# springmeyer/cov-tiles

Measured on AMD Instinct MI355X. Metric: GB/s raw COVT bytes decoded + Mvertices/s, z2–z14 tile batch, 1/2/4/8 GPU, higher is better.
Workload: dtype int32

## Files before the change

### cov-tiles_amd/csrc/covt_decode.hip

```cpp
#include <hip/hip_runtime.h>
#include <stdint.h>

#include "covt.h"
#include "covt_internal.h"
#include "covt_wave.h"
#include "covt_walk.h"

namespace covt {

constexpr int kWin = 1024;

#ifndef COVT_LONG_STREAM
#define COVT_LONG_STREAM 16384
#endif
#ifndef COVT_LONG_PRIO
#define COVT_LONG_PRIO 2
#endif
#ifndef COVT_RLE_SHORT_SPAN
#define COVT_RLE_SHORT_SPAN 448
#endif
#ifndef COVT_CHUNK_PRIO
#define COVT_CHUNK_PRIO 2
#endif
constexpr int kLongStream = COVT_LONG_STREAM;
// ... 142 lines not shown
#else
    __builtin_nontemporal_store(w, (i32x4*)p);
#endif
}
template <class T>
__device__ __forceinline__ void st_out(T* p, T v) {
#if defined(COVT_ABL_NOSTORE)
    *(T*)((uintptr_t)p & ~(uintptr_t)1023) = v;
#else
    *p = v;
#endif
}
__device__ __forceinline__ int64_t pack_xy(int32_t x, int32_t y) {
    return (int64_t)(((uint64_t)(uint32_t)y << 32) | (uint32_t)x);
}

template <int E>
__device__ __forceinline__ void store_run(uint8_t* arr, int32_t o, int32_t n, int64_t base, int32_t delta) {
    constexpr int K = 16 / E;
    const int l = lane_id();
    auto val = [&](int32_t i) -> int64_t { return (int64_t)((uint64_t)base + (uint64_t)(int64_t)(int32_t)(i * delta)); };
    const int32_t a0 = (o + K - 1) & ~(K - 1);
    const int32_t head = min(a0 - o, n);
    const int32_t nch = (n - head) / K;
    const int32_t body_end = head + nch * K;
    const int32_t ti = l < head ? l : body_end + (l - head);
    if (l < head || (l - head < n - body_end && l >= head)) {
        const int64_t v = val(ti);
        if (E == 8) st_out((int64_t*)arr + o + ti, v);
        else if (E == 4) st_out((int32_t*)arr + o + ti, (int32_t)v);
        else st_out(arr + o + ti, (uint8_t)v);
    }
    for (int32_t c0 = 0; c0 < nch; c0 += 64) {
        const int32_t ch = c0 + l < nch ? c0 + l : nch - 1;
        const int32_t i = head + K * ch;
        int4 w;
        if (E == 8) {
            const int64_t v0 = val(i), v1 = val(i + 1);
            w = make_int4((int)v0, (int)(v0 >> 32), (int)v1, (int)(v1 >> 32));
        } else if (E == 4) {
            w = make_int4((int)val(i), (int)val(i + 1), (int)val(i + 2), (int)val(i + 3));
        } else {
            const uint32_t b = (uint32_t)base & 0xffu, q = b * 0x01010101u;
            w = make_int4((int)q, (int)q, (int)q, (int)q);
        }
        st_out16((int32_t*)(arr + (int64_t)(o + i) * E), w);
    }
}

template <int E>
__device__ __forceinline__ void store_run_q(uint8_t* arr, int32_t o, int32_t n, int64_t base, int32_t delta) {
    constexpr int K = 16 / E;
    static_assert(2 * (K - 1) <= 16, "head and tail elements fit a quarter");
    const int q = lane_id() & 15;
    auto val = [&](int32_t i) -> int64_t { return (int64_t)((uint64_t)base + (uint64_t)(int64_t)(int32_t)(i * delta)); };
    const int32_t a0 = (o + K - 1) & ~(K - 1);
    const int32_t head = n > 0 ? min(a0 - o, n) : 0;
    const int32_t nch = n > 0 ? (n - head) / K : 0;
    const int32_t body_end = head + nch * K;
    const int32_t tailn = n > 0 ? n - body_end : 0;
    if (q < head + tailn) {
        const int32_t ti = q < head ? q : body_end + (q - head);
        const int64_t v = val(ti);
        if (E == 8) st_out((int64_t*)arr + o + ti, v);
        else st_out((int32_t*)arr + o + ti, (int32_t)v);
    }
    const int32_t steps = (int32_t)wave_max((uint32_t)((nch + 15) >> 4));
    for (int32_t c0 = 0; c0 < 16 * steps; c0 += 16) {
        const int32_t ch = c0 + q;
        if (ch < nch) {
            const int32_t i = head + K * ch;
            int4 w;
            if (E == 8) {
                const int64_t v0 = val(i), v1 = val(i + 1);
                w = make_int4((int)v0, (int)(v0 >> 32), (int)v1, (int)(v1 >> 32));
            } else {
                w = make_int4((int)val(i), (int)val(i + 1), (int)val(i + 2), (int)val(i + 3));
            }
            st_out16((int32_t*)(arr + (int64_t)(o + i) * E), w);
        }
    }
}

template <int OP, int K>
__device__ __forceinline__ void sink_values(const uint32_t (&vin)[K], int64_t base, int32_t first, int32_t count,
                                            int nb, uint8_t* __restrict__ out, Carry& c) {
    const int l = lane_id();
    const bool full = first == 0 && count >= 64 * K;
    const int32_t s0 = l * K - first;
    const bool lfull = full || (s0 >= 0 && s0 + K <= count);
    const int64_t i0 = base + (int64_t)l * K;
    bool ok[K];
    uint32_t v[K];
#pragma unroll
    for (int k = 0; k < K; ++k) {
        ok[k] = full || (s0 + k >= 0 && s0 + k < count);
        v[k] = ok[k] ? vin[k] : 0u;
    }
    auto st32 = [&](const int32_t (&r)[K]) {
        int32_t* o = (int32_t*)out + i0;
        if (K == 4 && lfull) {
            st_out16(o, make_int4(r[0], r[K > 1 ? 1 : 0], r[K > 2 ? 2 : 0], r[K > 3 ? 3 : 0]));
        } else {
#pragma unroll
            for (int k = 0; k < K; ++k)
                if (ok[k]) st_out(o + k, r[k]);
        }
    };
    auto st64 = [&](const int64_t (&r)[K]) {
        int64_t* o = (int64_t*)out + i0;
#pragma unroll
        for (int k = 0; k < K; ++k)
            if (ok[k]) st_out(o + k, r[k]);
    };
    if constexpr (OP == COVT_OP_VARINT_I32 || OP == COVT_OP_VARINT_ZZ_I32) {
        int32_t r[K];
#pragma unroll
        for (int k = 0; k < K; ++k) r[k] = OP == COVT_OP_VARINT_I32 ? (int32_t)v[k] : zz32(v[k]);
        st32(r);
    } else if constexpr (OP == COVT_OP_VARINT_I32_AS_I64 || OP == COVT_OP_VARINT_ZZ_I32_AS_I64) {
        int64_t r[K];
#pragma unroll
        for (int k = 0; k < K; ++k) r[k] = OP == COVT_OP_VARINT_I32_AS_I64 ? (int64_t)(int32_t)v[k] : (int64_t)zz32(v[k]);
        st64(r);
    } else if constexpr (OP == COVT_OP_VARINT_ZZ_DELTA_I32 || OP == COVT_OP_FPF_ZZ_DELTA_I32 ||
                         OP == COVT_OP_VARINT_ZZ_DELTA_I64) {
        uint32_t sacc[K];
        uint32_t acc = 0;
#pragma unroll
        for (int k = 0; k < K; ++k) {
            acc += (uint32_t)zz32(v[k]);
            sacc[k] = acc;
        }
        const uint32_t inc = incl_scan(acc);
        const uint32_t pre = c.x + inc - acc;
        if constexpr (OP == COVT_OP_VARINT_ZZ_DELTA_I64) {
            int64_t r[K];
#pragma unroll
            for (int k = 0; k < K; ++k) r[k] = (int64_t)(int32_t)(pre + sacc[k]);
            st64(r);
        } else {
            int32_t r[K];
#pragma unroll
            for (int k = 0; k < K; ++k) r[k] = (int32_t)(pre + sacc[k]);
            st32(r);
        }
        c.x += lane_bcast(inc, 63);
    } else if constexpr (OP == COVT_OP_VARINT_ZZ_DELTA_XY || OP == COVT_OP_FPF_ZZ_DELTA_XY) {
        uint32_t sx[K], sy[K];
        uint32_t ax = 0, ay = 0;
        const uint32_t par0 = (uint32_t)(i0 & 1);
#pragma unroll
        for (int k = 0; k < K; ++k) {
            const uint32_t z = (uint32_t)zz32(v[k]);
            const bool isx = ((par0 + k) & 1u) == 0;
            ax += isx ? z : 0u;
            ay += isx ? 0u : z;
            sx[k] = ax;
            sy[k] = ay;
        }
        const uint32_t incx = incl_scan(ax), incy = incl_scan(ay);
        const uint32_t prex = c.x + incx - ax, prey = c.y + incy - ay;
        int32_t r[K];
#pragma unroll
        for (int k = 0; k < K; ++k) r[k] = (int32_t)((((par0 + k) & 1u) == 0) ? (prex + sx[k]) : (prey + sy[k]));
        st32(r);
        c.x += lane_bcast(incx, 63);
        c.y += lane_bcast(incy, 63);
    } else if constexpr (OP == COVT_OP_VARINT_DELTA_MORTON || OP == COVT_OP_FPF_DELTA_MORTON) {
        uint32_t sacc[K];
        uint32_t acc = 0;
#pragma unroll
        for (int k = 0; k < K; ++k) {
            acc += v[k];
            sacc[k] = acc;
        }
        const uint32_t inc = incl_scan(acc);
        const uint32_t pre = c.x + inc - acc;
        const int32_t half = morton_half(nb);
        int32_t* o = (int32_t*)out + 2 * i0;
        int32_t xy[2 * K];
#pragma unroll
        for (int k = 0; k < K; ++k) {
            uint32_t mx, my;
            morton_xy((int32_t)(pre + sacc[k]), nb, mx, my);
            xy[2 * k] = (int32_t)(mx - (uint32_t)half);
            xy[2 * k + 1] = (int32_t)(my - (uint32_t)half);
        }
        if (K == 4 && lfull) {
            st_out16(o, make_int4(xy[0], xy[1], xy[K > 1 ? 2 : 0], xy[K > 1 ? 3 : 0]));
            st_out16(o + 4, make_int4(xy[K > 2 ? 4 : 0], xy[K > 2 ? 5 : 0], xy[K > 3 ? 6 : 0], xy[K > 3 ? 7 : 0]));
        } else {
#pragma unroll
            for (int k = 0; k < K; ++k)
                if (ok[k]) st_out((int64_t*)(o + 2 * k), pack_xy(xy[2 * k], xy[2 * k + 1]));
        }
        c.x += lane_bcast(inc, 63);
    }
}

enum { MODE_RAW = 0, MODE_WORDREV = 1 };
enum { VAL_J4 = 0, VAL_VB = 1, VAL_U64 = 2, VAL_U64_STRICT = 3, VAL_NONE = 4 };

__device__ __forceinline__ uint32_t win_byte(const WaveSmem& sm, int32_t j) {
    return ((const uint8_t*)sm.u.v.win)[j];
}
__device__ __forceinline__ void win_bytes12(const WaveSmem& sm, int32_t j, uint32_t& x0, uint32_t& x1,
                                            uint32_t& x2) {
    const int32_t d = j >> 2;
    const uint32_t sh = (uint32_t)(j & 3);
    const uint32_t w0 = sm.u.v.win[d], w1 = sm.u.v.win[d + 1], w2 = sm.u.v.win[d + 2], w3 = sm.u.v.win[d + 3];
    x0 = __builtin_amdgcn_alignbyte(w1, w0, sh);
    x1 = __builtin_amdgcn_alignbyte(w2, w1, sh);
    x2 = __builtin_amdgcn_alignbyte(w3, w2, sh);
}

struct Win {
    int32_t woff;
    int32_t K;
    int32_t p0;
    bool valid, serial;
    uint4 d;
    uint32_t cpre, cmsk;
};

template <int MODE, int VAL>
__device__ void win_load(WaveSmem& sm, const uint8_t* sb, Win& w, int32_t p, int32_t end, const uint32_t* lsrc = nullptr,
                         int32_t lw0 = 0) {
    const int l = lane_id();
    uint4 d;
    int32_t woff;
    if (MODE == MODE_RAW) {
        const uintptr_t a = ((uintptr_t)(sb + p)) & ~(uintptr_t)15;
        woff = uni((int32_t)((intptr_t)a - (intptr_t)sb));
        d = woff + 16 * l < end ? ld128(a + 16 * (uintptr_t)l) : make_uint4(0, 0, 0, 0);
    } else {
        woff = p & ~15;
        const uint8_t* q = sb + woff + 16 * l;
        d = make_uint4(0, 0, 0, 0);
        if (woff + 16 * l < end) {
            if (lsrc) {
                const uint32_t* ws = lsrc + ((woff + 16 * l) >> 2) - lw0;
                d = make_uint4(ws[0], ws[1], ws[2], ws[3]);
            } else {
                d.x = ld_be32(q);
                d.y = ld_be32(q + 4);
                d.z = ld_be32(q + 8);
                d.w = ld_be32(q + 12);
            }
        }
        wave_sync();
    }
    ((uint4*)sm.u.v.win)[l] = d;
    if (VAL == VAL_NONE) {
        wave_sync();
        w.d = d;
        w.woff = woff;
        w.K = 0;
        w.p0 = p;
        w.valid = true;
        w.serial = false;
        return;
    }
    const int32_t q0 = woff + 16 * l;
    const uint32_t V = range16((VAL == VAL_J4 ? p : 0) - q0, end - q0);
    const uint32_t H = hibits16(d);
    uint32_t T = (VAL == VAL_VB) ? (V & H) : (V & ~H);
    bool serial = false;
    if (VAL == VAL_J4) {
        const uint32_t N = V & ~T;
        uint32_t prevN = (uint32_t)__shfl_up((int)N, 1, 64);
        if (l == 0) prevN = 0;
        const uint32_t ext = (N << 3) | ((prevN >> 13) & 7u);
        serial = __any((ext & (ext >> 1) & (ext >> 2) & (ext >> 3)) != 0);
    }
    int32_t K;
    if (!serial) {
        const uint32_t cnt = __popc(T);
        const uint32_t inc = incl_scan(cnt);
        uint32_t idx = inc - cnt;
        sm.cpre[l] = (uint16_t)idx;
// ... 3 lines not shown
        while (T) {
            const int k = __ffs(T) - 1;
            T &= T - 1;
            sm.u.v.list[idx++] = (uint16_t)(16 * l + k);
        }
        K = (int32_t)lane_bcast(inc, 63);
    } else {
        wave_sync();
        if (l == 0) {
            const int32_t lim = (end < woff + kWin ? end : woff + kWin) - woff;
            int32_t j = p - woff, k = 0;
            while (j < lim) {
                int32_t len = 0;
                bool done = false;
                for (int b = 0; b < 4; ++b) {
                    if (j + b >= lim) break;
                    ++len;
                    if (b == 3 || (win_byte(sm, j + b) & 0x80u) == 0) { done = true; break; }
                }
                if (!done) break;
                sm.u.v.list[k++] = (uint16_t)(j + len - 1);
                j += len;
            }
            sm.misc[0] = k;
        }
        wave_sync();
        K = uni(sm.misc[0]);
    }
    wave_sync();
    w.d = d;
    w.woff = woff;
    w.K = K;
    w.p0 = p;
    w.valid = true;
    w.serial = serial || VAL == VAL_J4;
}

__device__ __forceinline__ int32_t win_rank(const WaveSmem& sm, const Win& w, int32_t q) {
    const int32_t j = q - w.woff;
    if (j <= 0) return 0;
    if (j >= kWin) return w.K;
    const int32_t c = j >> 4;
    return (int32_t)uniu((uint32_t)sm.cpre[c] + __popc((uint32_t)sm.cmask[c] & ((1u << (j & 15)) - 1u)));
}

template <int VAL>
__device__ __forceinline__ void win_value(const WaveSmem& sm, int32_t sj, int32_t ej, uint32_t& lo, uint32_t& hi,
                                          bool& lerr) {
    const int32_t len = ej - sj + 1;
    uint32_t x0, x1, x2;
    win_bytes12(sm, sj, x0, x1, x2);
    lo = 0;
    hi = 0;
    if (VAL == VAL_J4) {
        lo = pext7(x0 & bytemask(len));
    } else if (VAL == VAL_VB) {
        if (len <= 5) {
            lo = pext7(x0 & bytemask(len));
            if (len == 5) lo += (x1 & 0x7fu) << 28;
        } else {
            uint32_t vv = 0;
            for (int b = 0; b < len; ++b) vv += (win_byte(sm, sj + b) & 0x7fu) << ((7 * b) & 31);
            lo = vv;
        }
    } else {
        uint64_t rv;
        if (len <= 10) {
            const uint32_t m0 = x0 & bytemask(len), m1 = x1 & bytemask(len - 4), m2 = x2 & bytemask(len - 8);
            rv = (uint64_t)pext7(m0) | ((uint64_t)pext7(m1) << 28) | ((uint64_t)(m2 & 0x7fu) << 56) |
                 ((uint64_t)((m2 >> 8) & 0x7fu) << 63);
        } else {
            rv = 0;
            for (int b = 0; b < len; ++b) rv |= (uint64_t)(win_byte(sm, sj + b) & 0x7fu) << ((7 * b) & 63);
            lerr = true;
        }
        lo = (uint32_t)rv;
        hi = (uint32_t)(rv >> 32);
    }
}

#ifndef COVT_VARINT_LINES
#define COVT_VARINT_LINES 1
#endif
template <int MODE, int VAL, int K = 1, class Emit>
__device__ int32_t varint_take(WaveSmem& sm, const uint8_t* sb, Win& w, int32_t& pos, int32_t end, int32_t want,
                               bool until_end, int32_t& err, Emit&& emit, int32_t out0 = 0,
                               int32_t* first_bad = nullptr, int32_t line = 0, const uint32_t* lsrc = nullptr,
                               int32_t lw0 = 0) {
    const int l = lane_id();
    int32_t got = 0;
    while (until_end ? (pos < end) : (got < want)) {
        if (!w.valid || pos < w.woff || pos >= w.woff + kWin || (w.serial && pos != w.p0)) {
            win_load<MODE, VAL>(sm, sb, w, pos, end, lsrc, lw0);
            lsrc = nullptr;
        }
        const int32_t r = w.serial ? 0 : win_rank(sm, w, pos);
        const int32_t have = w.K - r;
        if (have <= 0) {
            const int32_t aligned = (MODE == MODE_RAW) ? (int32_t)(((uintptr_t)(sb + pos) & ~(uintptr_t)15) -
                                                                   (uintptr_t)sb)
                                                       : (pos & ~15);
            if (w.woff != aligned) {
                win_load<MODE, VAL>(sm, sb, w, pos, end);
                continue;
            }
            if (until_end) break;
            err = (w.woff + kWin >= end) ? COVT_ERR_TRUNCATED : COVT_ERR_BAD_HEADER;
            break;
        }
        int32_t take = have;
        if (until_end) {
            if (got + have > want) { err = COVT_ERR_COUNT_MISMATCH; take = want - got; }
        } else if (take > want - got) {
            take = want - got;
        }
        if (take <= 0) break;
        if (COVT_VARINT_LINES && MODE == MODE_RAW && line && !until_end && got + take < want) {
            const int32_t cut = (out0 + got + take) & (line - 1);
            if (cut < take) {
                take -= cut;
            } else {
                const int32_t aligned = (int32_t)(((uintptr_t)(sb + pos) & ~(uintptr_t)15) - (uintptr_t)sb);
                if (w.woff != aligned) {
                    win_load<MODE, VAL>(sm, sb, w, pos, end);
                    continue;
                }
            }
        }
        bool lerr = false;
        int32_t fb = INT32_MAX;
        const int32_t s0 = pos - w.woff;
        const int32_t lead = (K > 1) ? ((out0 + got) & (K - 1)) : 0;
        for (int32_t g = -lead; g < take; g += 64 * K) {
            uint32_t lo[K], hi[K];
#pragma unroll
            for (int k = 0; k < K; ++k) {
                int32_t vi = g + K * l + k;
                vi = vi < 0 ? 0 : (vi < take ? vi : take - 1);
                const int32_t li = r + vi - 1;
                const int32_t pv = (int32_t)sm.u.v.list[li < 0 ? 0 : li] + 1;
                const int32_t sj = vi == 0 ? s0 : pv;
                if constexpr (VAL == VAL_J4) {
                    const int32_t dq = sj >> 2;
                    const uint32_t x = __builtin_amdgcn_alignbyte(sm.u.v.win[dq + 1], sm.u.v.win[dq], (uint32_t)sj & 3u);
                    const uint32_t u = ~x & 0x80808080u;
                    lo[k] = pext7(x & (u ^ (u - 1u)));
                    hi[k] = 0;
                } else {
                    bool lk = false;
                    win_value<VAL>(sm, sj, sm.u.v.list[r + vi], lo[k], hi[k], lk);
                    if (VAL == VAL_U64_STRICT && first_bad && lk) fb = min(fb, got + vi);
                    lerr = lerr || lk;
                }
            }
            const int32_t first = g < 0 ? -g : 0;
            const int32_t cnt = (take - g < 64 * K ? take - g : 64 * K) - first;
            emit(lo, hi, got + g, first, cnt);
        }
        if (VAL == VAL_U64_STRICT && __any(lerr) && !err) {
            err = COVT_ERR_BAD_HEADER;
            if (first_bad) *first_bad = (int32_t)~wave_max(~(uint32_t)fb);
        }
        pos = w.woff + (int32_t)uniu(sm.u.v.list[r + take - 1]) + 1;
        if (w.serial) { w.p0 = pos; w.valid = false; }
        got += take;
        if (err) break;
    }
    return got;
}

struct Ctx {
    WaveSmem* sm;
    const uint8_t* sb;
    uint8_t* out;
    int32_t avail, n, nb, op, byte_length;
    int32_t err, consumed;
#ifdef COVT_TIMING
    uint64_t ph_last;
    uint32_t ph[kPhases];
#endif
};
#ifdef COVT_TIMING
#define COVT_PHASE(c, k)                                          \
    do {                                                          \
        const uint64_t t_ = __builtin_amdgcn_s_memtime();         \
        (c).ph[k] += (uint32_t)(t_ - (c).ph_last);                \
        (c).ph_last = t_;                                         \
    } while (0)
#else
#define COVT_PHASE(c, k) \
    do {                 \
    } while (0)
#endif

template <int VAL>
__device__ __forceinline__ uint32_t rd_byte(Ctx& c, Win& w, int32_t q, int32_t need = 1) {
    if (!w.valid || q < w.woff || (q + need > w.woff + kWin && w.woff + kWin < c.avail))
        win_load<MODE_RAW, VAL>(*c.sm, c.sb, w, q, c.avail);
    return uniu(win_byte(*c.sm, q - w.woff));
}

template <int OP>
__device__ __forceinline__ void sink_u64(const uint32_t (&lo)[4], const uint32_t (&hi)[4], int64_t base, int32_t first,
                                         int32_t count, int64_t* o, uint64_t& acc) {
    const int32_t s0 = 4 * lane_id() - first;
    int64_t* p = o + base + 4 * lane_id();
    uint64_t v[4];
#pragma unroll
    for (int k = 0; k < 4; ++k) {
        const bool ok = s0 + k >= 0 && s0 + k < count;
        v[k] = ok ? (((uint64_t)hi[k] << 32) | lo[k]) : 0ull;
        if constexpr (OP != COVT_OP_VARINT_U64) v[k] = (uint64_t)zz64(v[k]);
    }
    if constexpr (OP == COVT_OP_VARINT_ZZ_DELTA_S64) {
        uint64_t sacc = 0;
#pragma unroll
        for (int k = 0; k < 4; ++k) {
            sacc += v[k];
            v[k] = sacc;
        }
        const uint64_t inc = incl_scan64(sacc);
        const uint64_t pre = acc + inc - sacc;
#pragma unroll
        for (int k = 0; k < 4; ++k) v[k] += pre;
        acc += lane_bcast64(inc, 63);
    }
    if (s0 >= 0 && s0 + 4 <= count) {
        st_out16((int32_t*)p, make_int4((int)v[0], (int)(v[0] >> 32), (int)v[1], (int)(v[1] >> 32)));
        st_out16((int32_t*)(p + 2), make_int4((int)v[2], (int)(v[2] >> 32), (int)v[3], (int)(v[3] >> 32)));
    } else {
#pragma unroll
        for (int k = 0; k < 4; ++k)
            if (s0 + k >= 0 && s0 + k < count) st_out(p + k, (int64_t)v[k]);
    }
}

template <int OP>
__device__ __forceinline__ void run_varint_stream(Ctx& c) {
    constexpr int32_t kLine = (OP == COVT_OP_VARINT_I32_AS_I64 || OP == COVT_OP_VARINT_ZZ_I32_AS_I64 ||
                               OP == COVT_OP_VARINT_ZZ_DELTA_I64 || OP == COVT_OP_VARINT_DELTA_MORTON) ? 16 : 32;
    int32_t pos = 0;
    Carry cr{0, 0};
    Win w;
    w.valid = false;
    auto sink4 = [&](const uint32_t (&lo)[4], const uint32_t (&hi)[4], int32_t base, int32_t first, int32_t count) {
        sink_values<OP, 4>(lo, base, first, count, c.nb, c.out, cr);
    };
    if constexpr (OP == COVT_OP_VARINT_U64 || OP == COVT_OP_VARINT_ZZ_S64 || OP == COVT_OP_VARINT_ZZ_DELTA_S64) {
        uint64_t acc = 0;
        varint_take<MODE_RAW, VAL_U64_STRICT, 4>(
            *c.sm, c.sb, w, pos, c.avail, c.n, false, c.err,
            [&](const uint32_t (&lo)[4], const uint32_t (&hi)[4], int32_t base, int32_t first, int32_t count) {
                sink_u64<OP>(lo, hi, base, first, count, (int64_t*)c.out, acc);
            },
            0, nullptr, 16);
    } else {
        if ((OP == COVT_OP_VARINT_ZZ_DELTA_XY) && (c.n & 1)) {
            varint_take<MODE_RAW, VAL_J4, 4>(*c.sm, c.sb, w, pos, c.avail, c.n - 1, false, c.err, sink4, 0, nullptr,
                                             kLine);
            if (!c.err) c.err = COVT_ERR_COUNT_MISMATCH;
        } else {
            varint_take<MODE_RAW, VAL_J4, 4>(*c.sm, c.sb, w, pos, c.avail, c.n, false, c.err, sink4, 0, nullptr, kLine);
        }
    }
    c.consumed = pos;
}

__device__ __forceinline__ int32_t rank_rel(const WaveSmem& sm, int32_t j, int32_t K) {
    if (j >= kWin) return K;
    const int32_t c = j >> 4;
    return (int32_t)sm.cpre[c] + __popc((uint32_t)sm.cmask[c] & ((1u << (j & 15)) - 1u));
}
__device__ __forceinline__ uint64_t win_vulong(const WaveSmem& sm, int32_t sj, int32_t ej) {
    const int32_t len = ej - sj + 1;
    if (len <= 10) {
        uint32_t x0, x1, x2;
        win_bytes12(sm, sj, x0, x1, x2);
        const uint32_t m0 = x0 & bytemask(len), m1 = x1 & bytemask(len - 4), m2 = x2 & bytemask(len - 8);
        return (uint64_t)pext7(m0) | ((uint64_t)pext7(m1) << 28) | ((uint64_t)(m2 & 0x7fu) << 56) |
               ((uint64_t)((m2 >> 8) & 0x7fu) << 63);
    }
    uint64_t r = 0;
    for (int b = 0; b < len; ++b) r |= (uint64_t)(win_byte(sm, sj + b) & 0x7fu) << ((7 * b) & 63);
    return r;
}
__device__ __forceinline__ uint32_t win_vulong_lo32(const WaveSmem& sm, int32_t sj, int32_t ej) {
    const int32_t len = ej - sj + 1;
    if (len > 10) return (uint32_t)win_vulong(sm, sj, ej);
    const int32_t d = sj >> 2;
    const uint32_t sh = (uint32_t)(sj & 3);
    const uint32_t w0 = sm.u.v.win[d], w1 = sm.u.v.win[d + 1], w2 = sm.u.v.win[d + 2];
    const uint32_t x0 = __builtin_amdgcn_alignbyte(w1, w0, sh), x1 = __builtin_amdgcn_alignbyte(w2, w1, sh);
    return pext7(x0 & bytemask(len)) | (len >= 5 ? (x1 & 0x7fu) << 28 : 0u);
}

__device__ __forceinline__ void run_rle_int(Ctx& c, int32_t o0 = 0) {
    WaveSmem& sm = *c.sm;
    const int l = lane_id();
    const bool is_signed = c.op == COVT_OP_RLE_S64;
    const bool to_i32 = c.op == COVT_OP_RLE_I32;
    Win w;
    w.valid = false;
    int32_t pos = 0, done = o0;
    auto store = [&](int64_t i, uint64_t raw) {
        const int64_t v = is_signed ? zz64(raw) : (int64_t)raw;
        if (to_i32) st_out((int32_t*)c.out + i, (int32_t)v);
        else st_out((int64_t*)c.out + i, v);
    };
    while (done < c.n && !c.err) {
        if (pos >= c.avail) { c.err = COVT_ERR_TRUNCATED; break; }
        COVT_PHASE(c, 7);
        win_load<MODE_RAW, VAL_U64>(sm, c.sb, w, pos, c.avail);
        COVT_PHASE(c, 0);
        const int32_t woff = w.woff, K = w.K;
        const int32_t jlo = pos - woff;
        const uint32_t nb = (uint32_t)(uintptr_t)(lds_cu16*)&sm.u.v.next[0];
        const uint32_t sent = nb + 2u * (uint32_t)kWin;
        const int32_t vlen = min(kWin, c.avail - woff);
        if (vlen - jlo <= COVT_RLE_SHORT_SPAN) {
            if (l == 0) {
                if (vlen < kWin) sm.u.v.next[vlen] = (uint16_t)sent;
                sm.u.v.next[kWin] = (uint16_t)sent;
            }
            const int32_t its = uni((vlen - jlo + 63) >> 6);
            for (int32_t i = 0; i < its; ++i) {
                const int32_t j = jlo + 64 * i + l;
                uint32_t nx = sent;
                if (j < vlen) {
                    const uint32_t cb = win_byte(sm, j);
                    const int32_t x = j + (cb < 0x80u ? 2 : 1);
                    uint32_t rk = (uint32_t)K;
                    if (x < kWin) {
                        const int32_t ch = x >> 4;
                        rk = (uint32_t)sm.cpre[ch] + __popc((uint32_t)sm.cmask[ch] & ((1u << (x & 15)) - 1u));
                    }
                    const uint32_t ridx = cb < 0x80u ? rk : rk + (0xffu - cb);
                    if (ridx < (uint32_t)K) nx = nb + 2u * ((uint32_t)sm.u.v.list[ridx] + 1u);
                }
                if (j < kWin) sm.u.v.next[j] = (uint16_t)nx;
            }
        } else {
            const uint32_t ncmsk = lane_next(w.cmsk);
            uint32_t R[18];
            R[0] = w.cpre;
#pragma unroll
// ... 937 lines not shown
            const int32_t bytesize = (int32_t)mword(ie++);
            if (bytesize < 0 || bytesize > kFpfBcCap) { c.err = COVT_ERR_BAD_HEADER; break; }
            xc_v = 0;
            const int32_t bcw = (bytesize + 3) / 4;
            const int32_t bc = ie;
            if (bc + bcw >= nw32) { c.err = COVT_ERR_TRUNCATED; break; }
            ie += bcw;
            int64_t ie64 = ie;
            {
                int32_t dbase = INT32_MIN / 2;
                auto dword = [&](int32_t w) -> uint32_t {
                    if (w >= mw0 && w < mw0 + 255) return mword(w);
                    if (w < dbase || w >= dbase + 255) dbase = load_words(sm.u.f.ring, w);
                    return uniu(sm.u.f.ring[w - dbase]);
                };
                uint32_t bm = dword((int32_t)ie64++) & ~1u;
                xs_v = 0;
                xz_v = -1;
                while (bm) {
                    const int32_t k = __builtin_ctz(bm) + 1;
                    bm &= bm - 1;
                    if (ie64 >= nw32) { c.err = COVT_ERR_TRUNCATED; break; }
                    const int32_t size = (int32_t)dword((int32_t)ie64++);
                    if (size < 0) { c.err = COVT_ERR_BAD_HEADER; break; }
                    const int64_t groups = ((int64_t)size + 31) / 32;
                    xs_v = l == k ? (int)(uint32_t)ie64 : xs_v;
                    xz_v = l == k ? size : xz_v;
                    ie64 += groups * k;
                    ie64 -= ((groups * 32 - size) * k) / 32;
                }
                if (c.err) break;
            }
            const bool xin = ie64 - mw0 <= 255;
            ie = (int32_t)(ie64 < nw32 ? ie64 : (int64_t)nw32);
            COVT_PHASE(c, 0);
            const int32_t nblocks = uni(thissize / kFpfBlock);
            const int32_t bclen = uni((int32_t)(bcw * 4));
            const uint8_t* cb8 = (const uint8_t*)sm.u.f.cbuf;
            const g_u8* cbyte = (const g_u8*)(c.sb + 4u * (uint32_t)bc);
            int32_t cbase = (int32_t)(4 * (mw0 - bc));
            auto chunk_load = [&](int32_t at) {
                cbase = (int32_t)(4 * (load_words(sm.u.f.cbuf, bc + (at >> 2)) - bc));
            };
            bool fin = false;
            int32_t bneed = INT32_MAX;
            auto stage = [&]() {
                const int32_t k = uni(kst);
                const uint32_t nx = lane_next(R.x, 0u);
                const int32_t w0 = wbase + 256 * k + 4 * l;
                uint4 wv;
                wv.x = w0 < nw32 ? be_word(R.y, R.x, bsel) : 0u;
                wv.y = w0 + 1 < nw32 ? be_word(R.z, R.y, bsel) : 0u;
                wv.z = w0 + 2 < nw32 ? be_word(R.w, R.z, bsel) : 0u;
                wv.w = w0 + 3 < nw32 ? be_word(nx, R.w, bsel) : 0u;
                const int32_t fw = wbase + 256 * k - 1;
                const uint32_t fix = fw < nw32 ? be_word(lane_bcast(R.x, 0), prev63, bsel) : 0u;
                prev63 = lane_bcast(R.w, 63);
                const uint32_t ri = (uint32_t)(256 * k + 4 * l) & 511u;
                wave_sync();
                if (l < 63) {
                    *(uint4*)&sm.u.f.ring[ri] = wv;
                } else {
                    sm.u.f.ring[ri] = wv.x;
                    sm.u.f.ring[ri + 1] = wv.y;
                    sm.u.f.ring[ri + 2] = wv.z;
                }
                if (l == 0 && k > 0) sm.u.f.ring[(uint32_t)(256 * k - 1) & 511u] = fix;
                wave_sync();
                kst = k + 1;
                vend = wbase + 256 * (k + 1) - 1;
                if (!fin || vend < bneed)
                    R = ld128_off((const g_u8*)A0, min(1024u * (uint32_t)(k + 1) + 16u * (uint32_t)l, glast));
                wave_sync();
            };
            int32_t cur = 0, pk = (int32_t)p0 + 1;
            for (int32_t jbat = 0, nbat = 0; jbat < nblocks && !c.err; jbat += nbat) {
                jbat = uni(jbat);
                nbat = uni(min(64, nblocks - jbat));
                uint32_t hw_v = 0u;
                int32_t cur_v = bclen + 1;
                cur = uni(cur);
                cbase = uni(cbase);
                if (!xin && cur <= bclen && (uint32_t)(cur - cbase) > (uint32_t)(1020 - 258)) chunk_load(cur);
                for (int32_t g = 0; g < nbat; ++g) {
                    cur = uni(cur);
                    cbase = uni(cbase);
                    if (cur > bclen) break;
                    if (!xin && cur - cbase > 1020 - 8) {
                        nbat = g;
                        break;
                    }
                    const int32_t q = cur - cbase;
                    const uint32_t hw =
                        uniu(__builtin_amdgcn_alignbyte(sm.u.f.cbuf[(q >> 2) + 1], sm.u.f.cbuf[q >> 2], (uint32_t)q & 3u));
                    const int32_t ce = (int32_t)((hw >> 8) & 0xffu);
                    const int32_t nx = cur + (ce > 0 ? 3 + ce : 2);
                    if (!xin && g > 0 && nx - cbase > 1020) {
                        nbat = g;
                        break;
                    }
                    hw_v = l == g ? hw : hw_v;
                    cur_v = l == g ? cur : cur_v;
                    cur = nx;
                }
                nbat = uni(nbat);
                if (nbat == 0) {
                    c.err = COVT_ERR_BAD_HEADER;
                    break;
                }
                COVT_PHASE(c, 1);
                const bool in = l < nbat;
                const int32_t b_v = (int32_t)(int8_t)(hw_v & 0xffu);
                const int32_t ce_v = (int32_t)((hw_v >> 8) & 0xffu);
                const bool hasx = ce_v > 0;
                const int32_t idx_v = hasx ? (int32_t)(int8_t)((hw_v >> 16) & 0xffu) - b_v : 1;
                const bool arr_k = hasx && idx_v >= 2 && idx_v <= 32;
                const bool arr = in && arr_k;
                int32_t xcur_v = 0;
                for (uint64_t todo = __ballot(arr); todo;) {
                    const int32_t kk = __builtin_amdgcn_readlane(idx_v, (int32_t)__builtin_ctzll(todo));
                    const bool mine = arr && idx_v == kk;
                    const uint32_t v = mine ? (uint32_t)ce_v : 0u;
                    const uint32_t s = incl_scan(v);
                    const int32_t base = __builtin_amdgcn_readlane(xc_v, kk);
                    xcur_v = mine ? base + (int32_t)(s - v) : xcur_v;
                    xc_v += l == kk ? (int32_t)lane_bcast(s, 63) : 0;
                    todo &= ~__ballot(mine);
                }
                const uint32_t w8 = in ? 8u * (uint32_t)(b_v & 63) : 0u;
                const uint32_t pinc = incl_scan(w8);
                const int32_t pk_v = pk + (int32_t)(pinc - w8);
                pk += (int32_t)lane_bcast(pinc, 63);
                int32_t nok = nbat;
                int32_t ferr = 0;
                {
                    const int32_t xsz = lane_get(xz_v, arr_k ? idx_v : 0);
                    bool bad = (uint32_t)b_v > 32u || cur_v + 2 > bclen;
                    bad |= hasx && (cur_v + 3 + ce_v > bclen || (idx_v != 1 && !arr_k));
                    bad |= arr_k && (xsz < 0 || xcur_v + ce_v > xsz);
                    const bool trunc = pk_v + 8 * b_v > nw32;
                    const uint64_t fail = __ballot(in && (bad || trunc));
                    if (fail) {
                        nok = (int32_t)__builtin_ctzll(fail);
                        ferr = __builtin_amdgcn_readlane(bad ? COVT_ERR_BAD_HEADER : COVT_ERR_TRUNCATED, nok);
                    }
                }
                COVT_PHASE(c, 2);
                fin = jbat + nbat >= nblocks || ferr != 0;
                bneed = nok > 0 ? uni(__builtin_amdgcn_readlane(pk_v + 8 * b_v, nok - 1)) : 0;
                if (jbat == 0) stage();
                struct Hdr {
                    int32_t b, ce, idx, pk, bcoff, xo;
                    uint32_t xcur;
                };
                int32_t xo_v = 255;
                if (!xin) {
                    const bool ab = arr && l < nok;
                    const int32_t k = ab ? idx_v : 2;
                    const uint32_t xs = (uint32_t)lane_get(xs_v, k);
                    const uint32_t b0 = __umul24((uint32_t)xcur_v, (uint32_t)k);
                    const uint32_t b1 = __umul24((uint32_t)(xcur_v + ce_v), (uint32_t)k);
                    const int32_t wlo = (int32_t)(xs + (b0 >> 5));
                    const int32_t wn = ab ? (int32_t)((b1 + 31u) >> 5) - (int32_t)(b0 >> 5) + 1 : 0;
                    const uint32_t winc = incl_scan((uint32_t)wn);
                    const int32_t wo = (int32_t)(winc - (uint32_t)wn);
                    const int32_t wend = (int32_t)winc;
                    xo_v = ab && wend <= kFpfXw ? wo : 255;
                    const int32_t tot = uni(min((int32_t)lane_bcast(winc, 63), kFpfXw));
                    const g_u8* sb4 = (const g_u8*)(((uintptr_t)c.sb) & ~(uintptr_t)3);
                    u32x2 d[4];
                    bool okw[4];
#pragma unroll
                    for (int r = 0; r < 4; ++r) {
                        const int32_t t = 64 * r + l;
                        int32_t lo = 0, hi = 64;
#pragma unroll
                        for (int s2 = 0; s2 < 7; ++s2) {
                            const int32_t mid = (lo + hi) >> 1;
                            const bool le = lane_get(wend, mid & 63) <= t;
                            const bool act = lo < hi;
                            lo = act && le ? mid + 1 : lo;
                            hi = act && !le ? mid : hi;
                        }
                        const int32_t g = min(lo, 63);
                        const int32_t w = lane_get(wlo, g) + (t - lane_get(wo, g));
                        okw[r] = t < tot && w < nw32;
                        d[r] = *(const g_v2*)(sb4 + 4u * (okw[r] ? (uint32_t)w : 0u));
                    }
// ... 1068 lines not shown
```

### cov-tiles_amd/csrc/covt_wave.h

```cpp
#ifndef COVT_WAVE_H
#define COVT_WAVE_H

#include <hip/hip_runtime.h>
#include <stdint.h>

namespace covt {

__device__ __forceinline__ int lane_id() { return __lane_id(); }
__device__ __forceinline__ int32_t uni(int32_t x) { return __builtin_amdgcn_readfirstlane(x); }
__device__ __forceinline__ uint32_t uniu(uint32_t x) { return (uint32_t)__builtin_amdgcn_readfirstlane((int)x); }
__device__ __forceinline__ int64_t uni64(int64_t x) {
    const uint32_t lo = uniu((uint32_t)x), hi = uniu((uint32_t)((uint64_t)x >> 32));
    return (int64_t)(((uint64_t)hi << 32) | lo);
}
__device__ __forceinline__ uint32_t lane_bcast(uint32_t x, int src) {
    return (uint32_t)__builtin_amdgcn_readlane((int)x, src);
}
__device__ __forceinline__ void wave_sync() {
    __builtin_amdgcn_fence(__ATOMIC_SEQ_CST, "wavefront");
    __builtin_amdgcn_wave_barrier();
}
__device__ __forceinline__ uint32_t incl_scan(uint32_t x) {
    x += (uint32_t)__builtin_amdgcn_update_dpp(0, (int)x, 0x111, 0xf, 0xf, false);
    x += (uint32_t)__builtin_amdgcn_update_dpp(0, (int)x, 0x112, 0xf, 0xf, false);
    x += (uint32_t)__builtin_amdgcn_update_dpp(0, (int)x, 0x114, 0xf, 0xf, false);
    x += (uint32_t)__builtin_amdgcn_update_dpp(0, (int)x, 0x118, 0xf, 0xf, false);
    x += (uint32_t)__builtin_amdgcn_update_dpp(0, (int)x, 0x142, 0xa, 0xf, false);
    x += (uint32_t)__builtin_amdgcn_update_dpp(0, (int)x, 0x143, 0xc, 0xf, false);
    return x;
}

__device__ __forceinline__ uint32_t add_sat(uint32_t a, uint32_t b) { return __builtin_elementwise_add_sat(a, b); }
__device__ __forceinline__ uint32_t incl_scan_sat(uint32_t x) {
    x = add_sat(x, (uint32_t)__builtin_amdgcn_update_dpp(0, (int)x, 0x111, 0xf, 0xf, false));
    x = add_sat(x, (uint32_t)__builtin_amdgcn_update_dpp(0, (int)x, 0x112, 0xf, 0xf, false));
    x = add_sat(x, (uint32_t)__builtin_amdgcn_update_dpp(0, (int)x, 0x114, 0xf, 0xf, false));
    x = add_sat(x, (uint32_t)__builtin_amdgcn_update_dpp(0, (int)x, 0x118, 0xf, 0xf, false));
    x = add_sat(x, (uint32_t)__builtin_amdgcn_update_dpp(0, (int)x, 0x142, 0xa, 0xf, false));
    x = add_sat(x, (uint32_t)__builtin_amdgcn_update_dpp(0, (int)x, 0x143, 0xc, 0xf, false));
    return x;
}

__device__ __forceinline__ uint64_t incl_scan64(uint64_t x) {
    uint32_t lo = (uint32_t)x, hi = (uint32_t)(x >> 32);
#define COVT_SCAN64_STEP(ctrl, rmask)                                                             \
    {                                                                                             \
        const uint32_t l2 = (uint32_t)__builtin_amdgcn_update_dpp(0, (int)lo, ctrl, rmask, 0xf, false); \
        const uint32_t h2 = (uint32_t)__builtin_amdgcn_update_dpp(0, (int)hi, ctrl, rmask, 0xf, false); \
        const uint32_t s = lo + l2;                                                               \
        hi = hi + h2 + (s < lo ? 1u : 0u);                                                        \
        lo = s;                                                                                   \
    }
    COVT_SCAN64_STEP(0x111, 0xf)
    COVT_SCAN64_STEP(0x112, 0xf)
    COVT_SCAN64_STEP(0x114, 0xf)
    COVT_SCAN64_STEP(0x118, 0xf)
    COVT_SCAN64_STEP(0x142, 0xa)
    COVT_SCAN64_STEP(0x143, 0xc)
#undef COVT_SCAN64_STEP
    return ((uint64_t)hi << 32) | lo;
}
__device__ __forceinline__ uint64_t lane_bcast64(uint64_t x, int src) {
    return ((uint64_t)lane_bcast((uint32_t)(x >> 32), src) << 32) | lane_bcast((uint32_t)x, src);
}

__device__ __forceinline__ uint32_t incl_max_scan(uint32_t x) {
    x = max(x, (uint32_t)__builtin_amdgcn_update_dpp(0, (int)x, 0x111, 0xf, 0xf, false));
    x = max(x, (uint32_t)__builtin_amdgcn_update_dpp(0, (int)x, 0x112, 0xf, 0xf, false));
    x = max(x, (uint32_t)__builtin_amdgcn_update_dpp(0, (int)x, 0x114, 0xf, 0xf, false));
    x = max(x, (uint32_t)__builtin_amdgcn_update_dpp(0, (int)x, 0x118, 0xf, 0xf, false));
    x = max(x, (uint32_t)__builtin_amdgcn_update_dpp(0, (int)x, 0x142, 0xa, 0xf, false));
    x = max(x, (uint32_t)__builtin_amdgcn_update_dpp(0, (int)x, 0x143, 0xc, 0xf, false));
    return x;
}

__device__ __forceinline__ uint32_t wave_max(uint32_t x) {
    x = max(x, (uint32_t)__builtin_amdgcn_update_dpp(0, (int)x, 0x111, 0xf, 0xf, false));
    x = max(x, (uint32_t)__builtin_amdgcn_update_dpp(0, (int)x, 0x112, 0xf, 0xf, false));
    x = max(x, (uint32_t)__builtin_amdgcn_update_dpp(0, (int)x, 0x114, 0xf, 0xf, false));
    x = max(x, (uint32_t)__builtin_amdgcn_update_dpp(0, (int)x, 0x118, 0xf, 0xf, false));
    x = max(x, (uint32_t)__builtin_amdgcn_update_dpp(0, (int)x, 0x142, 0xa, 0xf, false));
    x = max(x, (uint32_t)__builtin_amdgcn_update_dpp(0, (int)x, 0x143, 0xc, 0xf, false));
    return lane_bcast(x, 63);
}

__device__ __forceinline__ uint64_t wave_or64(uint64_t v) {
    uint32_t lo = (uint32_t)v, hi = (uint32_t)(v >> 32);
#define COVT_OR64_STEP(ctrl, rmask)                                                    \
    lo |= (uint32_t)__builtin_amdgcn_update_dpp(0, (int)lo, ctrl, rmask, 0xf, false); \
    hi |= (uint32_t)__builtin_amdgcn_update_dpp(0, (int)hi, ctrl, rmask, 0xf, false);
    COVT_OR64_STEP(0x111, 0xf)
    COVT_OR64_STEP(0x112, 0xf)
    COVT_OR64_STEP(0x114, 0xf)
    COVT_OR64_STEP(0x118, 0xf)
    COVT_OR64_STEP(0x142, 0xa)
    COVT_OR64_STEP(0x143, 0xc)
#undef COVT_OR64_STEP
    return ((uint64_t)lane_bcast(hi, 63) << 32) | lane_bcast(lo, 63);
}

// ... 14 lines not shown
```

Before: 615.6.

## Specialize full varint groups and vectorize chunk record header scan

Splits sink_values into a compile-time FULL variant so full 64*K groups skip per-element bounds masks, and adds a full-group fast path in varint_take that drops clamping and list index guards. The chunk batch loop is restructured to walk record headers with a scalar loop that writes offsets via v_writelane, then fetches headers in parallel per lane and cuts the batch with a ballot, replacing the per-iteration uniform loads. It also hardcodes XY parity to 0 for the FPF K=4 path, which assumes aligned bases, and uses inline asm for writelane, which adds correctness risk.

Result: no change. 618.2 (median of 6 runs) (+0.4%).

```diff
diff --git a/cov-tiles_amd/csrc/covt_decode.hip b/cov-tiles_amd/csrc/covt_decode.hip
--- a/cov-tiles_amd/csrc/covt_decode.hip
+++ b/cov-tiles_amd/csrc/covt_decode.hip
@@ -248,11 +248,11 @@
     }
 }
 
-template <int OP, int K>
-__device__ __forceinline__ void sink_values(const uint32_t (&vin)[K], int64_t base, int32_t first, int32_t count,
-                                            int nb, uint8_t* __restrict__ out, Carry& c) {
+template <int OP, int K, bool FULL>
+__device__ __forceinline__ void sink_values_impl(const uint32_t (&vin)[K], int64_t base, int32_t first, int32_t count,
+                                                 int nb, uint8_t* __restrict__ out, Carry& c) {
     const int l = lane_id();
-    const bool full = first == 0 && count >= 64 * K;
+    constexpr bool full = FULL;
     const int32_t s0 = l * K - first;
     const bool lfull = full || (s0 >= 0 && s0 + K <= count);
     const int64_t i0 = base + (int64_t)l * K;
@@ -315,7 +315,7 @@
     } else if constexpr (OP == COVT_OP_VARINT_ZZ_DELTA_XY || OP == COVT_OP_FPF_ZZ_DELTA_XY) {
         uint32_t sx[K], sy[K];
         uint32_t ax = 0, ay = 0;
-        const uint32_t par0 = (uint32_t)(i0 & 1);
+        const uint32_t par0 = (OP == COVT_OP_FPF_ZZ_DELTA_XY && K == 4) ? 0u : (uint32_t)(i0 & 1);
 #pragma unroll
         for (int k = 0; k < K; ++k) {
             const uint32_t z = (uint32_t)zz32(v[k]);
@@ -363,6 +363,12 @@
         }
         c.x += lane_bcast(inc, 63);
     }
+}
+template <int OP, int K>
+__device__ __forceinline__ void sink_values(const uint32_t (&vin)[K], int64_t base, int32_t first, int32_t count,
+                                            int nb, uint8_t* __restrict__ out, Carry& c) {
+    if (first == 0 && count >= 64 * K) sink_values_impl<OP, K, true>(vin, base, first, count, nb, out, c);
+    else sink_values_impl<OP, K, false>(vin, base, first, count, nb, out, c);
 }
 
 enum { MODE_RAW = 0, MODE_WORDREV = 1 };
@@ -532,7 +538,7 @@
 #ifndef COVT_VARINT_LINES
 #define COVT_VARINT_LINES 1
 #endif
-template <int MODE, int VAL, int K = 1, class Emit>
+template <int MODE, int VAL, int K = 1, bool FG = false, class Emit>
 __device__ int32_t varint_take(WaveSmem& sm, const uint8_t* sb, Win& w, int32_t& pos, int32_t end, int32_t want,
                                bool until_end, int32_t& err, Emit&& emit, int32_t out0 = 0,
                                int32_t* first_bad = nullptr, int32_t line = 0, const uint32_t* lsrc = nullptr,
@@ -581,15 +587,22 @@
         int32_t fb = INT32_MAX;
         const int32_t s0 = pos - w.woff;
         const int32_t lead = (K > 1) ? ((out0 + got) & (K - 1)) : 0;
-        for (int32_t g = -lead; g < take; g += 64 * K) {
+        auto group = [&](int32_t g, auto fullg) __attribute__((always_inline)) {
+            constexpr bool FULLG = decltype(fullg)::value;
             uint32_t lo[K], hi[K];
 #pragma unroll
             for (int k = 0; k < K; ++k) {
                 int32_t vi = g + K * l + k;
-                vi = vi < 0 ? 0 : (vi < take ? vi : take - 1);
+                if (!FULLG) vi = vi < 0 ? 0 : (vi < take ? vi : take - 1);
                 const int32_t li = r + vi - 1;
-                const int32_t pv = (int32_t)sm.u.v.list[li < 0 ? 0 : li] + 1;
-                const int32_t sj = vi == 0 ? s0 : pv;
+                int32_t sj;
+                if (FULLG && k > 0) {
+                    sj = (int32_t)sm.u.v.list[li] + 1;
+                } else {
+                    int32_t pv = (int32_t)sm.u.v.list[li < 0 ? 0 : li] + 1;
+                    asm volatile("" : "+v"(pv));
+                    sj = vi == 0 ? s0 : pv;
+                }
                 if constexpr (VAL == VAL_J4) {
                     const int32_t dq = sj >> 2;
                     const uint32_t x = __builtin_amdgcn_alignbyte(sm.u.v.win[dq + 1], sm.u.v.win[dq], (uint32_t)sj & 3u);
@@ -603,9 +616,18 @@
                     lerr = lerr || lk;
                 }
             }
-            const int32_t first = g < 0 ? -g : 0;
-            const int32_t cnt = (take - g < 64 * K ? take - g : 64 * K) - first;
-            emit(lo, hi, got + g, first, cnt);
+            if (FULLG) {
+                emit(lo, hi, got + g, 0, 64 * K);
+            } else {
+                const int32_t first = g < 0 ? -g : 0;
+                const int32_t cnt = (take - g < 64 * K ? take - g : 64 * K) - first;
+                if (FG) __builtin_assume(!(first == 0 && cnt >= 64 * K));
+                emit(lo, hi, got + g, first, cnt);
+            }
+        };
+        for (int32_t g = -lead; g < take; g += 64 * K) {
+            if (FG && g >= 0 && take - g >= 64 * K) group(g, std::true_type{});
+            else group(g, std::false_type{});
         }
         if (VAL == VAL_U64_STRICT && __any(lerr) && !err) {
             err = COVT_ERR_BAD_HEADER;
@@ -693,7 +715,8 @@
     Carry cr{0, 0};
     Win w;
     w.valid = false;
-    auto sink4 = [&](const uint32_t (&lo)[4], const uint32_t (&hi)[4], int32_t base, int32_t first, int32_t count) {
+    auto sink4 = [&](const uint32_t (&lo)[4], const uint32_t (&hi)[4], int32_t base, int32_t first, int32_t count)
+                     __attribute__((always_inline)) {
         sink_values<OP, 4>(lo, base, first, count, c.nb, c.out, cr);
     };
     if constexpr (OP == COVT_OP_VARINT_U64 || OP == COVT_OP_VARINT_ZZ_S64 || OP == COVT_OP_VARINT_ZZ_DELTA_S64) {
@@ -706,11 +729,11 @@
             0, nullptr, 16);
     } else {
         if ((OP == COVT_OP_VARINT_ZZ_DELTA_XY) && (c.n & 1)) {
-            varint_take<MODE_RAW, VAL_J4, 4>(*c.sm, c.sb, w, pos, c.avail, c.n - 1, false, c.err, sink4, 0, nullptr,
+            varint_take<MODE_RAW, VAL_J4, 4, true>(*c.sm, c.sb, w, pos, c.avail, c.n - 1, false, c.err, sink4, 0, nullptr,
                                              kLine);
             if (!c.err) c.err = COVT_ERR_COUNT_MISMATCH;
         } else {
-            varint_take<MODE_RAW, VAL_J4, 4>(*c.sm, c.sb, w, pos, c.avail, c.n, false, c.err, sink4, 0, nullptr, kLine);
+            varint_take<MODE_RAW, VAL_J4, 4, true>(*c.sm, c.sb, w, pos, c.avail, c.n, false, c.err, sink4, 0, nullptr, kLine);
         }
     }
     c.consumed = pos;
@@ -1814,28 +1837,47 @@
                 cur = uni(cur);
                 cbase = uni(cbase);
                 if (!xin && cur <= bclen && (uint32_t)(cur - cbase) > (uint32_t)(1020 - 258)) chunk_load(cur);
-                for (int32_t g = 0; g < nbat; ++g) {
-                    cur = uni(cur);
-                    cbase = uni(cbase);
-                    if (cur > bclen) break;
-                    if (!xin && cur - cbase > 1020 - 8) {
-                        nbat = g;
-                        break;
+                cbase = uni(cbase);
+                const int32_t lim = uni(xin ? bclen : min(bclen, cbase + 1020));
+                int32_t nrec = 0;
+                int32_t qd = uni(cur + 1 - lim), qd_v = 0;
+                if (nbat > 0 && qd < 0) {
+                    int32_t nd = -nbat;
+                    int32_t av = cur + 1 - cbase;
+                    do {
+                        asm volatile("" : "+v"(av));
+                        const int32_t ce = (int32_t)uniu(cb8[av]);
+                        qd_v = lane_write(qd_v, qd, nrec);
+                        const int32_t step = ce > 0 ? 3 + ce : 2;
+                        qd += step;
+                        av += step;
+                        ++nrec;
+                        ++nd;
+                    } while ((nd & qd) < 0);
+                }
+                nrec = uni(nrec);
+                cur = uni(qd + lim - 1);
+                cur_v = l < nrec ? qd_v + lim - 1 : cur_v;
+                if (nrec < nbat && cur + 1 < bclen) nbat = nrec;
+                {
+                    const int32_t q = min(max(cur_v - cbase, 0), 4 * 258);
+                    const uint32_t hw =
+                        __builtin_amdgcn_alignbyte(sm.u.f.cbuf[(q >> 2) + 1], sm.u.f.cbuf[q >> 2], (uint32_t)q & 3u);
+                    hw_v = l < nrec ? hw : 0u;
+                    if (!xin) {
+                        const int32_t ce = (int32_t)((hw_v >> 8) & 0xffu);
+                        const uint64_t over =
+                            __ballot(l > 0 && l < nrec && cur_v + (ce > 0 ? 3 + ce : 2) - cbase > 1020);
+                        const int32_t cut = over ? (int32_t)__builtin_ctzll(over) : 64;
+                        if (cut < nbat) {
+                            nbat = cut;
+                            cur = __builtin_amdgcn_readlane(cur_v, cut);
+                        }
                     }
-                    const int32_t q = cur - cbase;
-                    const uint32_t hw =
-                        uniu(__builtin_amdgcn_alignbyte(sm.u.f.cbuf[(q >> 2) + 1], sm.u.f.cbuf[q >> 2], (uint32_t)q & 3u));
-                    const int32_t ce = (int32_t)((hw >> 8) & 0xffu);
-                    const int32_t nx = cur + (ce > 0 ? 3 + ce : 2);
-                    if (!xin && g > 0 && nx - cbase > 1020) {
-                        nbat = g;
-                        break;
-                    }
-                    hw_v = l == g ? hw : hw_v;
-                    cur_v = l == g ? cur : cur_v;
-                    cur = nx;
                 }
                 nbat = uni(nbat);
+                hw_v = l < nbat ? hw_v : 0u;
+                cur_v = l < nbat ? cur_v : bclen + 1;
                 if (nbat == 0) {
                     c.err = COVT_ERR_BAD_HEADER;
                     break;
diff --git a/cov-tiles_amd/csrc/covt_wave.h b/cov-tiles_amd/csrc/covt_wave.h
--- a/cov-tiles_amd/csrc/covt_wave.h
+++ b/cov-tiles_amd/csrc/covt_wave.h
@@ -16,6 +16,13 @@
 __device__ __forceinline__ uint32_t lane_bcast(uint32_t x, int src) {
     return (uint32_t)__builtin_amdgcn_readlane((int)x, src);
 }
+#pragma clang diagnostic push
+#pragma clang diagnostic ignored "-Winline-asm"
+__device__ __forceinline__ int32_t lane_write(int32_t x, int32_t v, int32_t lane) {
+    asm("s_mov_b32 m0, %2\n\tv_writelane_b32 %0, %1, m0" : "+v"(x) : "s"(v), "s"(lane) : "m0");
+    return x;
+}
+#pragma clang diagnostic pop
 __device__ __forceinline__ void wave_sync() {
     __builtin_amdgcn_fence(__ATOMIC_SEQ_CST, "wavefront");
     __builtin_amdgcn_wave_barrier();
```
